# thanh-nt25/Whisper-context-biasing

Hardware: AMD Instinct MI355X
Metric: audio-seconds/sec (RTF) + biased-WER, whisper-small 30s clips, batch32 (higher is better)
Workload: dtype bf16

## Files before the change

### include/wcb.h

```cpp
#ifndef WCB_H_
#define WCB_H_
#include <stdint.h>

#ifdef __cplusplus
extern "C" {
#endif

typedef struct wcb_handle wcb_handle;
typedef struct wcb_bias wcb_bias;

enum wcb_status {
  WCB_OK = 0,
  WCB_ERR_ARG = -1,
  WCB_ERR_STATE = -2,
  WCB_ERR_HIP = -3,
  WCB_ERR_UNSUPPORTED = -4
};

enum wcb_dtype { WCB_BF16 = 0, WCB_F16 = 1, WCB_F32 = 2 };

typedef struct {
  int d_model, n_layers, n_heads, ffn, vocab, n_mel;
  int n_audio_ctx;
  int n_text_ctx;
// ... 47 lines not shown
int wcb_decode_info(wcb_handle* h, wcb_state* st, int32_t* max_new, int32_t* steps, int32_t* done);
int wcb_decode_result(wcb_handle* h, wcb_state* st, int32_t* out_ids, int out_ld, int32_t* out_steps, void* stream);
int wcb_decode_end(wcb_handle* h, wcb_state* st);

int wcb_synchronize(wcb_handle* h);

int wcb_forward(wcb_handle* h, const float* mel, int B, const int32_t* dec_ids, int T, float* logits,
                void* enc_out, void* stream);

int wcb_forward_enc(wcb_handle* h, const void* enc, int B, const int32_t* dec_ids, int T, float* logits, void* stream);

int wcb_forward_cached(wcb_handle* h, wcb_state* st, const int32_t* dec_ids, int T, float* logits, void* stream);

int wcb_bias_create(wcb_handle* h, const int32_t* tokens, const int32_t* offsets, int n_phrases,
                    const uint8_t* word_start, wcb_bias** out);
void wcb_bias_destroy(wcb_bias* b);
int wcb_bias_num_states(const wcb_bias* b);

int wcb_profile_enable(wcb_handle* h, int enable);
int wcb_profile_read(wcb_handle* h, int n, char (*names)[32], int64_t* launches, double* ms,
                     double* flops, double* bytes);

int wcb_profile_kernel(wcb_handle* h, int i, char* name, int cap, int64_t* grid);

int wcb_debug_copy(wcb_handle* h, const char* name, void* dst, int64_t bytes, int enc_layers);

int wcb_op_gemm(int dtype, const void* A, const void* W, int M, int N, int K, const float* bias, int act,
                const float* resid, void* out, int out_f32, void* stream);
int wcb_op_gemm_kernel(int dtype, const void* A, const void* W, int M, int N, int K, const float* bias, int act,
                       const float* resid, void* out, int out_f32, int kernel, void* stream);
int wcb_op_gemm_ln(int dtype, const float* X, const float* ln_w, const float* ln_b, const float* stats,
                   const void* W, int M, int N, int K, const float* bias, int act, void* out, int out_f32,
                   void* stream);
int wcb_op_layernorm(int dtype, const float* x, const float* w, const float* b, void* y, int M, int d,
                     void* stream);
int wcb_op_attention(int dtype, const void* q, const void* k, const void* v, void* o, int B, int H, int Sq,
                     int Sk, int flash, void* stream);
int wcb_op_attention_decode(int dtype, const void* q, const void* k, const void* v, void* o, int B, int H,
                            int Sk, int nsplit, int variant, void* stream);

int wcb_op_cross_attention_enc(int dtype, const void* q, const void* enc, const void* wkt, const void* wv,
                               const float* bv, void* o, int B, int H, int S, int nsplit, int variant, void* stream);

int wcb_op_weighted_ce(const float* logits, long ld, int B, int T, int V, const int32_t* labels,
                       const int32_t* spans, const int32_t* span_len, int N, int Lmax, float bias_weight,
                       float* per_token, float* loss, int32_t* count, void* stream);

int wcb_wer_counts(const char* const* refs, const char* const* hyps, int n, int64_t* errors, int64_t* ref_words,
                   int n_threads);
int wcb_bias_counts(const char* ref, const char* pred, const char* const* phrases, int n_phrases,
                    int64_t* distance, int64_t* tokens);

#ifdef __cplusplus
}
#endif
#endif
```

### whisper_context_biasing_amd/_lib.py

```python
from __future__ import annotations

import ctypes as C
import os
import subprocess

_HERE = os.path.dirname(os.path.abspath(__file__))
LIB_PATH = os.path.join(_HERE, "libwcb.so")
CSRC = os.path.join(_HERE, "csrc")

WCB_BF16, WCB_F16, WCB_F32 = 0, 1, 2
DTYPES = {"bf16": WCB_BF16, "f16": WCB_F16, "fp16": WCB_F16, "f32": WCB_F32, "fp32": WCB_F32}


class WcbModelDesc(C.Structure):
    _fields_ = [(n, C.c_int) for n in (
        "d_model", "n_layers", "n_heads", "ffn", "vocab", "n_mel", "n_audio_ctx", "n_text_ctx",
        "eos_token_id", "pad_token_id", "decoder_start_token_id", "dtype")]


class WcbGenCfg(C.Structure):
    _fields_ = [("max_new_tokens", C.c_int), ("min_new_tokens", C.c_int), ("num_beams", C.c_int),
                ("bias_boost", C.c_float), ("use_graph", C.c_int), ("async_out", C.c_int)]


# ... 15 lines not shown
    "wcb_generate": (C.c_int, [_P, _P, C.c_int, C.POINTER(WcbGenCfg), _P, _P, C.c_int, _P,
                               C.POINTER(C.c_int32), _P]),
    "wcb_synchronize": (C.c_int, [_P]),
    "wcb_decode_begin": (C.c_int, [_P, _P, C.c_int, C.c_int, _P, C.c_int, C.c_float, C.c_int, C.POINTER(_P), _P]),
    "wcb_decode_step": (C.c_int, [_P, _P, _P, _P, _P, _P]),
    "wcb_decode_end": (C.c_int, [_P, _P]),
    "wcb_decode_begin_beams": (C.c_int, [_P, _P, C.c_int, C.c_int, _P, C.c_int, C.c_int, C.c_float, C.c_int,
                                         C.POINTER(_P), _P]),
    "wcb_decode_parents": (C.c_int, [_P, _P, _P, _P]),
    "wcb_decode_info": (C.c_int, [_P, _P, C.POINTER(C.c_int32), C.POINTER(C.c_int32), C.POINTER(C.c_int32)]),
    "wcb_decode_result": (C.c_int, [_P, _P, _P, C.c_int, C.POINTER(C.c_int32), _P]),
    "wcb_forward": (C.c_int, [_P, _P, C.c_int, _P, C.c_int, _P, _P, _P]),
    "wcb_forward_enc": (C.c_int, [_P, _P, C.c_int, _P, C.c_int, _P, _P]),
    "wcb_forward_cached": (C.c_int, [_P, _P, _P, C.c_int, _P, _P]),
    "wcb_bias_create": (C.c_int, [_P, _P, _P, C.c_int, _P, C.POINTER(_P)]),
    "wcb_bias_destroy": (None, [_P]),
    "wcb_bias_num_states": (C.c_int, [_P]),
    "wcb_debug_copy": (C.c_int, [_P, C.c_char_p, _P, C.c_int64, C.c_int]),
    "wcb_profile_enable": (C.c_int, [_P, C.c_int]),
    "wcb_profile_read": (C.c_int, [_P, C.c_int, _P, _P, _P, _P, _P]),
    "wcb_profile_kernel": (C.c_int, [_P, C.c_int, C.c_char_p, C.c_int, C.POINTER(C.c_int64)]),
    "wcb_op_gemm": (C.c_int, [C.c_int, _P, _P, C.c_int, C.c_int, C.c_int, _P, C.c_int, _P, _P,
                              C.c_int, _P]),
    "wcb_op_gemm_kernel": (C.c_int, [C.c_int, _P, _P, C.c_int, C.c_int, C.c_int, _P, C.c_int, _P, _P,
                                     C.c_int, C.c_int, _P]),
    "wcb_op_gemm_ln": (C.c_int, [C.c_int, _P, _P, _P, _P, _P, C.c_int, C.c_int, C.c_int, _P, C.c_int, _P,
                                 C.c_int, _P]),
    "wcb_op_weighted_ce": (C.c_int, [_P, C.c_long, C.c_int, C.c_int, C.c_int, _P, _P, _P, C.c_int, C.c_int,
                                     C.c_float, _P, _P, _P, _P]),
    "wcb_wer_counts": (C.c_int, [C.POINTER(C.c_char_p), C.POINTER(C.c_char_p), C.c_int,
                                 C.POINTER(C.c_int64), C.POINTER(C.c_int64), C.c_int]),
    "wcb_bias_counts": (C.c_int, [C.c_char_p, C.c_char_p, C.POINTER(C.c_char_p), C.c_int,
                                  C.POINTER(C.c_int64), C.POINTER(C.c_int64)]),
    "wcb_op_layernorm": (C.c_int, [C.c_int, _P, _P, _P, _P, C.c_int, C.c_int, _P]),
    "wcb_op_attention_decode": (C.c_int, [C.c_int, _P, _P, _P, _P, C.c_int, C.c_int, C.c_int, C.c_int, C.c_int,
                                          _P]),
    "wcb_op_attention": (C.c_int, [C.c_int, _P, _P, _P, _P, C.c_int, C.c_int, C.c_int, C.c_int,
                                   C.c_int, _P]),
    "wcb_op_cross_attention_enc": (C.c_int, [C.c_int, _P, _P, _P, _P, _P, _P, C.c_int, C.c_int, C.c_int,
                                             C.c_int, C.c_int, _P]),
    "wcb_set_option": (C.c_int, [_P, C.c_char_p, C.c_int]),
}


class WcbError(RuntimeError):
    pass


class WcbArgError(WcbError, ValueError):
    """WCB_ERR_ARG: the reference raises ValueError for these (e.g. whisper_medical.py:87-90)."""


_lib = None


def build(force: bool = False, jobs: int = 8) -> str:
    if force or not os.path.exists(LIB_PATH):
        subprocess.run(["make", "-C", CSRC, f"-j{jobs}"], check=True)
    return LIB_PATH


def load() -> C.CDLL:
    global _lib
    if _lib is not None:
        return _lib
    if not os.path.exists(LIB_PATH):
# ... 19 lines not shown
```

### whisper_context_biasing_amd/csrc/gemm_impl.h

```cpp
#pragma once
#include <stdexcept>
#include <string>
#include "common.h"
#include "kernels.h"

#include <algorithm>
#include <cstdio>
#include <cstdlib>
#include <type_traits>

namespace wcb {

WCB_DEV void glds16(const void* gptr, void* lds_wave_base) {
  __builtin_amdgcn_global_load_lds(gptr, (__attribute__((address_space(3))) void*)lds_wave_base, 16, 0, 0);
}

WCB_DEV long a_row(const GemmArgs& g, int m) {
  return g.a_Mb ? (long)(m / g.a_Mb) * g.a_strideB + (long)(m % g.a_Mb) * g.lda : (long)m * g.lda;
}
WCB_DEV long c_row(const GemmArgs& g, int m) {
  return g.c_Mb ? (long)(m / g.c_Mb) * g.c_strideB + (long)(m % g.c_Mb) * g.ldc : (long)m * g.ldc;
}

enum : int { E_BIAS = 1, E_GELU = 2, E_RESID = 4, E_F32 = 8, E_ADDROW = 16, E_HEAD = 32, E_RUNTIME = 1 << 30 };
// ... 1960 lines not shown
#pragma unroll
    for (int e = 0; e < 8; ++e) {
      float v;
      if constexpr (__is_same(T, bf16_t)) v = bf16_to_f((bf16_t)a[ks][e]);
      else v = float(a[ks][e]);
      xv[ks][e] = v;
      s1 += v;
      s2 = fmaf(v, v, s2);
    }
  }
  s1 = xor16_add(s1); s2 = xor16_add(s2);
  s1 = xor32_add(s1); s2 = xor32_add(s2);
  if (lane < 16) rst[wave][lane] = float2{s1, s2};
  __syncthreads();
  s1 = 0.f; s2 = 0.f;
#pragma unroll
  for (int q = 0; q < NW; ++q) { const float2 t = rst[q][lane & 15]; s1 += t.x; s2 += t.y; }
  const float mean = s1 / K;
  const float rstd = rsqrtf(fmaxf(s2 / K - mean * mean, 0.f) + 1e-5f);
  if (r >= M) return;
#pragma unroll
  for (int ks = 0; ks < KPW; ++ks) {
    Frag o;
#pragma unroll
    for (int e = 0; e < 8; ++e) {
      const float gwe = e < 4 ? w[ks][0][e] : w[ks][1][e - 4], gbe = e < 4 ? b[ks][0][e] : b[ks][1][e - 4];
      const float v = (xv[ks][e] - mean) * rstd * gwe + gbe;
      o[e] = __builtin_bit_cast(typename std::remove_reference<decltype(o[0])>::type, DT<T>::fromf(v));
    }
    *reinterpret_cast<Frag*>(out + (long)r * K + kb + ks * 32) = o;
  }
}

template <typename T, int MF, int NW, int KPW, int AM>
static void launch_dec_k(const GemmArgs& g, hipStream_t s) {
  const int ntile = (g.N + 15) / 16, gy = (g.M + MF * 16 - 1) / (MF * 16);
  if (!g.sel_val && (AM == 3 || ntile * gy <= 1024)) {
    WCB_LAUNCH((gemm_dec_kernel<T, MF, NW, KPW, AM, false>), dim3(ntile, gy), dim3(NW * 64), 0, s, g);
  } else {
    const int gx = std::min(ntile, g.walkers > 0 ? g.walkers : kDecWalkers);
    int nw = 0, kpw = 0;
    if constexpr (sizeof(T) == 2 && AM != 3) {
      if (g.W_fm && lean_cfg(g.K, nw, kpw) && nw == NW && kpw == KPW) {
        if (AM == 2 && g.ln_scratch && g.sel_val && g.a_Mb == 0) {
          WCB_LAUNCH((ln_rows_kernel<T, NW, KPW>), dim3((g.M + 15) / 16), dim3(NW * 64), 0, s,
                     reinterpret_cast<const T*>(g.ln_a16), g.lda, g.ln_w, g.ln_b, reinterpret_cast<T*>(g.ln_scratch), g.M);
          GemmArgs h = g;
          h.A = g.ln_scratch; h.lda = g.K;
          h.ln_w = h.ln_b = nullptr; h.ln_a16 = nullptr; h.st_in = nullptr;
          WCB_LAUNCH((gemm_dec_kernel<T, MF, NW, KPW, 0, true, true>), dim3(gx, gy), dim3(NW * 64), 0, s, h);
          return;
        }
        WCB_LAUNCH((gemm_dec_kernel<T, MF, NW, KPW, AM, true, true>), dim3(gx, gy), dim3(NW * 64), 0, s, g);
        return;
      }
    }
    WCB_LAUNCH((gemm_dec_kernel<T, MF, NW, KPW, AM == 3 ? 0 : AM, true>), dim3(gx, gy), dim3(NW * 64), 0, s, g);
  }
}

template <typename T, int MF, int NW, int KPW>
static bool launch_dec_am(const GemmArgs& g, hipStream_t s) {
  constexpr int K = NW * KPW * 32;
  if (g.ln_w) {
    if constexpr (K <= 1280) {
      if (g.ln_a16) launch_dec_k<T, MF, NW, KPW, 2>(g, s);
      else launch_dec_k<T, MF, NW, KPW, 1>(g, s);
      return true;
    }
    return false;
  }
  if (g.a_grp_n) {
    if constexpr (K <= 1280) {
      launch_dec_k<T, MF, NW, KPW, 3>(g, s);
      return true;
    }
    return false;
  }
  launch_dec_k<T, MF, NW, KPW, 0>(g, s);
  return true;
}

template <typename T, int MF>
static bool launch_dec_mf(const GemmArgs& g, hipStream_t s) {
// ... 141 lines not shown
```

### whisper_context_biasing_amd/csrc/kernels.h

```cpp
#pragma once
#include <hip/hip_runtime.h>
#include <hip/hip_ext.h>
#include <stdint.h>

namespace wcb {

struct LaunchTimer {
  hipEvent_t start = nullptr, stop = nullptr;
  int n = 0;
  const void* fn = nullptr;
  long grid = 0;
};
inline thread_local LaunchTimer g_launch_timer;

#define WCB_LAUNCH(K, G, B, SH, S, ...)                                                              \
  do {                                                                                               \
    ::wcb::LaunchTimer& lt_ = ::wcb::g_launch_timer;                                                 \
    if (lt_.stop) {                                                                                  \
      if (!lt_.n) {                                                                                  \
        lt_.fn = reinterpret_cast<const void*>(K);                                                   \
        const dim3 g_ = dim3(G), b_ = dim3(B);                                                       \
        lt_.grid = (long)g_.x * g_.y * g_.z * b_.x * b_.y * b_.z;                                    \
      }                                                                                              \
      hipExtLaunchKernelGGL(K, G, B, SH, S, lt_.n ? nullptr : lt_.start, lt_.stop, 0, __VA_ARGS__);  \
// ... 22 lines not shown
  const int* pos = nullptr; int kv_T = 0;
  void* kv_out = nullptr; int n_split = 0;
  int kv_rps = 0;
  int tile = 0;
  const float* st_in = nullptr;
  float* st_out = nullptr;
  int st_nb = 0;
  float* sel_val = nullptr; int* sel_idx = nullptr;
  const uint32_t* sel_root_bits = nullptr; float sel_lam = 0.f;
  const int* sel_rowbase = nullptr;
  int sel_eos = -1; const int* sel_step = nullptr; int sel_min_new = 0;
  int a_grp_n = 0; long a_grp_off = 0;
  int skinny = 0;
  int ring_kt = 1;
  int wide = 0;
  int walkers = 0;
  void* out16 = nullptr;
  const void* ln_a16 = nullptr;
  const float* ln_u = nullptr;
  const float* ln_c = nullptr;
  const void* ln_wg = nullptr;
  const void* ln_wg_fm = nullptr;
  int lean_fold = 0;
  int lean_mf2 = 0;
  const void* xqk_wk = nullptr; void* xqk_out = nullptr; int xqk_nch = 0;
  const float* rst_in = nullptr; int rst_nb = 0;
  float* rst_out = nullptr;
  float clamp = 0.f;
  int lean = 0;
  const void* W_fm = nullptr;
  int c_fm = 0, a_fm = 0;
  void* out16_fm = nullptr;
  void* ln_scratch = nullptr;
  int raster = 0;
  int pp = 0;
  unsigned long long* kq_cnt = nullptr; int* kq_err = nullptr;
  const void* kq_w = nullptr; void* kq_out = nullptr; long kq_ld = 0;
  struct Stamp* lstamp = nullptr;
};

void gemm(DType t, const GemmArgs& g, hipStream_t s);
constexpr int kLnfMaxK = 1280;

void layernorm(DType t, const float* x, const float* w, const float* b, void* y, int M, int d,
               hipStream_t s);

void embed(DType t, const void* emb, const void* pos_emb, const int* ids, const int* pos, float* x,
           float* stats, int M, int d, hipStream_t s, void* x16 = nullptr, int V = 1 << 30, int rps = 1, int st_w = 16,
           void* x16fm = nullptr);
void prefill_ids(int* ids, const int* src, int R, int np, int ld, const int* pos, hipStream_t s);
void add_i32(int* p, int v, hipStream_t s);
constexpr int kDecWalkers = 512;
bool gemm_dec_supported(DType t, int K);
int lm_head_partials(DType t, int K, int vocab, int walkers = kDecWalkers);

constexpr int kStampSub = 64;
struct Stamp {
  unsigned long long* base = nullptr; const int* pos = nullptr; int stride = 0, idx = 0;
};

struct AttnArgs {
  const void* q = nullptr; long ldq = 0; long q_Sb = 0; int Sq = 1;
  const void* k = nullptr; const void* v = nullptr; long k_sb = 0, k_sh = 0, k_sk = 0;
  void* o = nullptr; long ldo = 0; long o_Sb = 0;
  int B = 0, H = 0;
  int nkeys = 0; const int* nkeys_dev = nullptr; int nkeys_add = 0;
// ... 140 lines not shown
```

### whisper_context_biasing_amd/csrc/runtime.cpp

```cpp
#include <hip/hip_runtime.h>

#include <algorithm>
#include <cxxabi.h>
#include <cmath>
#include <cstdio>
#include <cstring>
#include <map>
#include <thread>
#include <memory>
#include <stdexcept>
#include <string>
#include <vector>
#include <cstdlib>
#include <deque>
#include <atomic>

#include "../../include/wcb.h"
#include "kernels.h"

using namespace wcb;

namespace {

struct WcbError : std::runtime_error {
// ... 47 lines not shown
  float *lnx_w = nullptr, *lnx_b = nullptr;
  void* fc1_w = nullptr; float* fc1_b = nullptr;
  void* fc2_w = nullptr; float* fc2_b = nullptr;
  float *ln2_w = nullptr, *ln2_b = nullptr;
  void *qkv_wg = nullptr, *xq_wg = nullptr, *fc1_wg = nullptr;
  float *ln1_u = nullptr, *ln1_c = nullptr, *lnx_u = nullptr, *lnx_c = nullptr, *ln2_u = nullptr, *ln2_c = nullptr;
  void* xkt_w = nullptr; void* xv_w = nullptr; float* xv_b = nullptr;
  void *qkv_fm = nullptr, *o_fm = nullptr, *xq_fm = nullptr, *xkt_fm = nullptr, *xo_fm = nullptr, *fc1_fm = nullptr,
       *fc2_fm = nullptr;
  void* xv_fm = nullptr;
  void *qkv_wgfm = nullptr, *xq_wgfm = nullptr, *fc1_wgfm = nullptr;
};

struct ProfEntry {
  std::string name;
  int64_t launches = 0;
  double ms = 0, flops = 0, bytes = 0;
  const void* fn = nullptr;
  long grid = 0;
};

}

struct wcb_bias {
  int n_states = 1;
  int vocab = 0;
  uint64_t id = 0;
  wcb_handle* owner = nullptr;
  DevBuf root_bits, root_child, trans_off, trans_tok, trans_dst;
  DevBuf st_depth, st_keep;
};

static const char* const kLeanStampClass[] = {"dec_xattn", "dec_qkv", "dec_out", "dec_xq", "dec_xo", "dec_fc1", "dec_fc2",
                                              "dec_kq"};
static int lean_stamp_region(const char* cls) {
  for (int r = 1; r < 8; ++r)
    if (!strcmp(cls, kLeanStampClass[r])) return r;
  return 0;
}

struct DecCtx {
  static constexpr int kMaxSub = 8;
  hipStream_t hs = nullptr;
  hipStream_t sub[kMaxSub] = {};
  hipEvent_t ev_fork = nullptr, ev_join[kMaxSub] = {};
  int dec_B = 0, dec_T = 0;
  DevBuf kvself, dx, dx16, dx16fm, dh, dq, dqp, du, datt, dffn, dstats, drst, xpart, xml, xticket, logits, part_val, part_idx, ints,
      pids, outbuf, forced, beam;
  DevBuf kq_cnt;
  int nchunk = 64;
  hipGraphExec_t gexec = nullptr;
  hipGraphExec_t gexec_k = nullptr;
  int* done_h = nullptr;
  hipEvent_t ev_poll[2] = {};
  std::string gkey;
};

struct wcb_handle {
  wcb_model_desc d{};
  DType dt = kBF16;
  int device = 0;
  std::string err;
  hipStream_t he = nullptr;
  static constexpr int kMaxCtx = 4;
  int nctx = 2;
  hipEvent_t ev_xkv[kMaxCtx] = {}, ev_dec[kMaxCtx] = {};
  int gen_count = 0;
  hipEvent_t ev_in = nullptr, ev_out = nullptr;
  static constexpr int kMaxSub = DecCtx::kMaxSub;
  DecCtx dc[kMaxCtx];
  int n_sub = 1;
  int xsplit = 1;
  int xvariant = 0;
  int flash_split = 2;
  int beam_xattn = 0;
  int ln_fold = 1;
  int merge_v = 1;
  int xpart16 = 1;
  int xq_kq = 0;
  int ring_kt = 2;
  int beam_wide = 1;
  int beam_wfm = 0;
  int lean_fold = 1;
  int xqk = 1;
  int xqk_nch = 8;
  int merge_os = 1;
  int lm_walkers = 256;
  int mel_split = 0;
  int lean_mf2 = 0;
  int beam_chunks = 0;
  int beam_raster = 0;
  int lm_ln_split = 0;
  int enc_flash_qw = 4;
  int xmode = 1;
  int beam_xmode = 0;
  int group_rows = 512;
  int xenc_split = 6;
  int xenc_fm = 1;
  int xenc_variant = 1;
  int ln16 = 1;
  int vocab_pad = 0;
  int steps_per_graph = 8;
  int lean = 1;
  int lean_x = 1;
  struct wcb_state* step_state = nullptr;
  int enc_raster = 8;
  int enc_gemm = 4;
  bool dec_gemm = false;
  std::map<std::string, DevBuf> staged;
  std::vector<DevBuf> owned;
  bool ready = false;
  int dbg_enc_layers = -1;
  void *conv1_w = nullptr, *conv2_w = nullptr;
  float *conv1_b = nullptr, *conv2_b = nullptr, *enc_pos = nullptr;
  int k1pad = 0;
  std::vector<LayerW> enc, dec;
  float *enc_ln_w = nullptr, *enc_ln_b = nullptr, *dec_ln_w = nullptr, *dec_ln_b = nullptr;
  void* xkv_w = nullptr; float* xkv_b = nullptr;
  void *tok_emb = nullptr, *dec_pos = nullptr;
  void* tok_emb_fm = nullptr;
  DevBuf dft, dft3, mel_lo, mel_hi, mel_w, clip_max;
  int enc_B = 0;
  DevBuf xt, hbuf, x, h, qkv, att, ffn, encout;
  DevBuf xkv2[kMaxCtx];
  std::unique_ptr<wcb_bias> empty_bias;
  std::vector<wcb_bias*> biases;
  DevBuf dev_err;
  bool prof = false, prof_stamps = false;
  std::vector<ProfEntry> prof_e;
  std::deque<std::pair<int, std::pair<hipEvent_t, hipEvent_t>>> prof_pending;
  std::vector<hipEvent_t> ev_pool;
  DevBuf stamps, stamp_acc;
  static constexpr int kStampRegions = 8;
  unsigned long long* stamp_base(int buf, int region) {
    return stamps.as<unsigned long long>() + ((size_t)buf * kStampRegions + region) * stamp_slots() * 2 * kStampSub;
  }
  double xattn_bytes = 0, xattn_flops = 0;
  long stamp_slots() const { return (long)d.n_text_ctx * d.n_layers * kMaxSub; }

  int H() const { return d.n_heads; }
  int S() const { return d.n_audio_ctx; }

  void* upload(const void* src, size_t bytes) {
    owned.emplace_back();
    owned.back().ensure(bytes);
    HIPCHK(hipMemcpy(owned.back().p, src, bytes, hipMemcpyHostToDevice));
    return owned.back().p;
  }
  float* upload_f(const std::vector<float>& v) { return reinterpret_cast<float*>(upload(v.data(), v.size() * 4)); }
  void* own(size_t bytes) {
    owned.emplace_back();
    owned.back().ensure(bytes);
    return owned.back().p;
  }
  const float* W(const std::string& name, size_t expect) {
    auto it = staged.find(name);
    if (it == staged.end()) throw WcbError(WCB_ERR_STATE, "missing weight " + name);
    if (it->second.bytes != expect * 4)
      throw WcbError(WCB_ERR_ARG, "weight " + name + " has " + std::to_string(it->second.bytes / 4) +
                                      " elements, expected " + std::to_string(expect));
    return it->second.as<float>();
  }

  int prof_id(const char* name) {
    for (size_t i = 0; i < prof_e.size(); ++i)
      if (prof_e[i].name == name) return (int)i;
// ... 262 lines not shown
    REQUIRE(h && name, "bad argument");
    const std::string n = name;
    static const char* const kFreeWhileStepwise[] = {"decode_contexts", "enc_flash", "enc_gemm", "enc_raster",
                                                     "steps_per_graph", "kq_cnt_seed"};
    bool free_opt = false;
    for (const char* f : kFreeWhileStepwise) free_opt |= n == f;
    REQUIRE(free_opt || !h->step_state, "option " + n + ": a step-wise decode is active (wcb_decode_end first)");
    if (n == "xmode" || n == "beam_xmode") {
      REQUIRE(!h->ready, "option " + n + " selects the weight layouts: set it before wcb_finalize_weights");
      REQUIRE(value == 0 || value == 1, "option " + n + ": 0 or 1");
      if (n == "xmode") h->xmode = value && xenc_supported(h->dt, h->d.d_model);
      else h->beam_xmode = value && h->xmode;
      if (!h->xmode) h->beam_xmode = 0;
    } else if (n == "decode_contexts") {
      REQUIRE(value >= 1 && value <= wcb_handle::kMaxCtx, "option decode_contexts: 1..4");
      REQUIRE(!h->step_state || value < wcb_handle::kMaxCtx,
              "option decode_contexts: 4 while a step-wise decode is active (wcb_decode_end first)");
      h->nctx = value;
    } else if (n == "group_rows") {
      REQUIRE(value >= 16 && value <= 512, "option group_rows: 16..512");
      h->group_rows = value;
    } else if (n == "xenc_variant") {
      REQUIRE(value >= 0 && value <= 3, "option xenc_variant: 0..3");
      h->xenc_variant = value;
    } else if (n == "enc_flash") {
      REQUIRE(value == 2 || value == 4, "option enc_flash: 2 or 4");
      h->enc_flash_qw = value;
    } else if (n == "xenc_split") {
      REQUIRE(!h->ready, "option xenc_split: set before the weights are finalized");
      REQUIRE(value >= 1 && value <= kXencMaxSplit, "option xenc_split: 1..16");
      h->xenc_split = value;
    } else if (n == "lm_ln_split") {
      h->lm_ln_split = value != 0;
    } else if (n == "ring_kt") {
      REQUIRE(value == 1 || value == 2, "option ring_kt: 1 or 2");
      h->ring_kt = value;
    } else if (n == "kq_cnt_seed") {
      REQUIRE(value >= 0, "option kq_cnt_seed: >= 0");
      quiesce(h);
      for (DecCtx& D : h->dc) {
        if (!D.kq_cnt.p) continue;
        std::vector<unsigned long long> v(D.kq_cnt.bytes / 8, 4ull * (unsigned long long)value);
        HIPCHK(hipMemcpy(D.kq_cnt.p, v.data(), v.size() * 8, hipMemcpyHostToDevice));
      }
    } else if (n == "steps_per_graph") {
      REQUIRE(value >= 1 && value <= 64, "option steps_per_graph: 1..64");
      h->steps_per_graph = value;
    } else if (n == "xenc_fm") {
      h->xenc_fm = value != 0;
    } else if (n == "xq_kq") {
      h->xq_kq = value != 0;
    } else if (n == "enc_gemm") {
      REQUIRE(value == 0 || value == 1 || value == 4 || value == 5, "option enc_gemm: 0, 1, 4 or 5");
      h->enc_gemm = value;
    } else if (n == "enc_raster") {
      REQUIRE(value >= 0 && value <= 64, "option enc_raster: 0..64");
      h->enc_raster = value;
    } else if (n == "lean") {
      REQUIRE(!h->ready, "option lean selects weight layouts: set it before wcb_finalize_weights");
      h->lean = value != 0;
    } else if (n == "lean_x") {
      h->lean_x = value != 0;
    } else if (n == "xpart16") {
      h->xpart16 = value != 0;
    } else if (n == "merge_v") {
      h->merge_v = value != 0;
// ... 700 lines not shown
    xo.out16_fm = x16fm;
    proj("dec_xo", xo);
    const bool afm = fm_ok && w.fc1_fm && w.fc2_fm &&
                     (d == 512 || d == 768 || d == 1024 || d == 1280) &&
                     (h->d.ffn == 2048 || h->d.ffn == 3072 || h->d.ffn == 4096 || h->d.ffn == 5120);
    GemmArgs f1 = drow(x, d, w.fc1_w, M, h->d.ffn, d, dffn, h->d.ffn);
    f1.ln_w = w.ln2_w; f1.ln_b = w.ln2_b; f1.st_in = st; f1.st_nb = nbk; f1.ln_a16 = lna;
    f1.bias = w.fc1_b; f1.act = 1; f1.ln_u = w.ln2_u; f1.ln_c = w.ln2_c; f1.ln_wg = w.fc1_wg; f1.W_fm = w.fc1_fm; f1.ln_wg_fm = w.fc1_wgfm;
    f1.c_fm = afm;
    if (x16fm) { f1.ln_a16 = x16fm; f1.a_fm = 1; }
    proj("dec_fc1", f1);
    GemmArgs f2 = drow(dffn, h->d.ffn, w.fc2_w, M, d, h->d.ffn, x, d);
    f2.bias = w.fc2_b; f2.resid = x; f2.out_f32 = 1; f2.st_out = st_pub; f2.st_nb = nbk; f2.out16 = x16; f2.W_fm = w.fc2_fm;
    f2.a_fm = afm;
    f2.out16_fm = x16fm;
    proj("dec_fc2", f2);
  }
  if (c.lm_head) {
    GemmArgs lm = drow(x, d, h->tok_emb, M, h->d.vocab, d, c.logits_out + (size_t)b0 * c.logits_ld, c.logits_ld);
    if (rps > 1) { lm.ldc = h->d.vocab; lm.c_Mb = rps; lm.c_strideB = c.logits_ld; }
    const bool lm_tiled = tiled && rps == 1 && c.logits_ld >= h->vocab_pad;
    if (lm_tiled) lm.N = h->vocab_pad;
    lm.ln_w = h->dec_ln_w; lm.ln_b = h->dec_ln_b; lm.st_in = st; lm.st_nb = nbk; lm.ln_a16 = lna;
    if (h->lean) lm.W_fm = h->tok_emb_fm;
    if (h->lean && !tiled && rps == 1 && h->lm_ln_split) lm.ln_scratch = dh;
    lm.out_f32 = 1;
    if (c.select && !c.beam) {
      lm.walkers = h->lm_walkers;
      lm.sel_val = D.part_val.as<float>() + (size_t)b0 * D.nchunk;
      lm.sel_idx = D.part_idx.as<int>() + (size_t)b0 * D.nchunk;
      lm.sel_root_bits = c.bias->root_bits.as<uint32_t>(); lm.sel_lam = c.lam;
      lm.sel_rowbase = ints + I_NEXT + 3 * c.B + b0;
      lm.sel_eos = h->d.eos_token_id; lm.sel_step = ints + I_STEP; lm.sel_min_new = c.min_new;
    }
    if (lm_tiled) {
      proj("lm_head", lm);
    } else {
      dgemm(h, "lm_head", lm, st_);
    }
  }
}

void step_embed(wcb_handle* h, const StepCfg& c) {
  DecCtx& D = h->dc[c.buf];
  const int d = h->d.d_model, B = c.B;
  int* ints = D.ints.as<int>();
  const bool r32 = h->dec_gemm && lnf_possible(h);
  h->timed("dec_embed", 0, (double)B * d * (2.0 * esize(h->d.dtype) + 4), D.hs, [&] {
    embed(h->dt, h->tok_emb, h->dec_pos, ints + I_NEXT, ints + I_POS, D.dx.as<float>(),
          !h->dec_gemm ? D.dstats.as<float>() : r32 ? D.drst.as<float>() : nullptr, B, d, D.hs, D.dx16.p, h->d.vocab, 1,
          r32 ? 32 : 16, xfm_possible(h) ? D.dx16fm.p : nullptr);
  });
}

void decode_step(wcb_handle* h, const StepCfg& c) {
  DecCtx& D = h->dc[c.buf];
  const int d = h->d.d_model, B = c.B;
  int* ints = D.ints.as<int>();
  int* pos = ints + I_POS;
  int* next_ids = ints + I_NEXT;
  if (!c.embedded) step_embed(h, c);
  const int ngrp = (B + h->group_rows - 1) / h->group_rows;
  const int ns = std::max(ngrp, std::max(1, std::min(h->n_sub, B)));
  if (ns == 1 || !D.sub[0]) {
    for (int i = 0; i < ns; ++i) {
      const int b0 = (int)((long)B * i / ns), b1 = (int)((long)B * (i + 1) / ns);
// ... 870 lines not shown
    GemmArgs g = rowgemm(A, K, W, M, N, K, out, N);
    g.bias = bias; g.act = act; g.resid = resid; g.out_f32 = out_f32;
    g.raster = 8;
    if (kernel >= 6) {
      REQUIRE(M > 64 && dtype != WCB_F32, "decode-row tiles: 16-bit, M > 64");
      g.tile = 2; g.ring_kt = 2;
      if (kernel == 7) g.raster = 0;
      if (kernel <= 7 && wfm) g.W_fm = W;
      if (kernel > 7) {
        g.wide = kernel;
        if (wfm) g.W_fm = W;
        REQUIRE(!resid || resid == out, "wide tiles: the residual is updated in place (resid == out)");
      }
    } else {
      g.pp = kernel;
    }
    gemm(DType(dtype), g, (hipStream_t)stream);
    HIPCHK(hipGetLastError());
  });
}

int wcb_op_gemm(int dtype, const void* A, const void* W, int M, int N, int K, const float* bias, int act,
                const float* resid, void* out, int out_f32, void* stream) {
  return wcb_op_gemm_kernel(dtype, A, W, M, N, K, bias, act, resid, out, out_f32, 1, stream);
}

int wcb_op_gemm_ln(int dtype, const float* X, const float* ln_w, const float* ln_b, const float* stats,
                   const void* W, int M, int N, int K, const float* bias, int act, void* out, int out_f32, void* stream) {
  return guarded(nullptr, [&] {
    REQUIRE(X && ln_w && ln_b && stats && W && out && M > 0 && M <= 64 && N > 0 && K % 16 == 0, "bad argument");
    GemmArgs g = rowgemm(X, K, W, M, N, K, out, N);
    g.ln_w = ln_w; g.ln_b = ln_b; g.st_in = stats; g.st_nb = K / 16;
    g.bias = bias; g.act = act; g.out_f32 = out_f32;
    gemm(DType(dtype), g, (hipStream_t)stream);
    HIPCHK(hipGetLastError());
  });
}

int wcb_op_layernorm(int dtype, const float* x, const float* w, const float* b, void* y, int M, int d, void* stream) {
  return guarded(nullptr, [&] {
    REQUIRE(x && w && b && y && M > 0 && d > 0 && d % 64 == 0 && d <= 2048, "bad argument");
    layernorm(DType(dtype), x, w, b, y, M, d, (hipStream_t)stream);
    HIPCHK(hipGetLastError());
  });
}

int wcb_op_attention_decode(int dtype, const void* q, const void* k, const void* v, void* o, int B, int H, int Sk,
                            int nsplit, int variant, void* stream) {
  return guarded(nullptr, [&] {
    REQUIRE(q && k && v && o && B > 0 && H > 0 && Sk > 0 && Sk <= 2048 && nsplit >= 1 && nsplit <= 64, "bad argument");
    AttnArgs a;
    a.q = q; a.ldq = (long)H * 64; a.q_Sb = 1; a.Sq = 1;
    a.k = k; a.v = v; a.k_sb = (long)H * Sk * 64; a.k_sh = (long)Sk * 64; a.k_sk = 64;
    a.o = o; a.ldo = (long)H * 64; a.o_Sb = 1; a.B = B; a.H = H; a.nkeys = Sk;
    a.variant = variant;
    if (variant == 6 || variant == 7) a.kv_rows = Sk;
    int* nk_dev = nullptr;
    if (variant == 7) {
      HIPCHK(hipMallocAsync(reinterpret_cast<void**>(&nk_dev), 4, (hipStream_t)stream));
      const int nk1 = Sk - 1;
      write_i32(nk_dev, &nk1, 1, (hipStream_t)stream);
      a.nkeys_dev = nk_dev; a.nkeys_add = 1;
    }
    static DevBuf part, ticket;
    if (nsplit > 1) {
      a.nsplit = nsplit;
// ... 101 lines not shown
```

Measured before the change: 20400.

## Add streaming LM-head kernel with fused LayerNorm, bias boost and argmax select

Adds a dedicated lm_stream_kernel for the decoder LM head in greedy/select mode. It keeps the normalized activations in LDS, streams the vocab weight tiles with nontemporal loads through a multi-deep register ring, and fuses the bias boost, EOS masking and per-block argmax into the GEMM. The kernel is enabled by default through a new lm_stream option, and a standalone op entry point plus a profiling stamp region are added. The aim is to cut the memory-bound cost of reading the large vocab matrix each decode step. The cost is heavy register and LDS use, which may lower occupancy.

```diff
diff --git a/include/wcb.h b/include/wcb.h
--- a/include/wcb.h
+++ b/include/wcb.h
@@ -103,6 +103,10 @@
 int wcb_op_gemm_ln(int dtype, const float* X, const float* ln_w, const float* ln_b, const float* stats,
                    const void* W, int M, int N, int K, const float* bias, int act, void* out, int out_f32,
                    void* stream);
+int wcb_op_lm_head_select(int dtype, const void* A, const float* ln_w, const float* ln_b, void* ln_scratch,
+                          const void* W_fm, int M, int N, int K, const uint32_t* root_bits, const int32_t* rowbase,
+                          float lam, int eos, const int32_t* step, int min_new, int walkers, int kernel,
+                          float* part_val, int32_t* part_idx, float* logits, void* stream);
 int wcb_op_layernorm(int dtype, const float* x, const float* w, const float* b, void* y, int M, int d,
                      void* stream);
 int wcb_op_attention(int dtype, const void* q, const void* k, const void* v, void* o, int B, int H, int Sq,
diff --git a/whisper_context_biasing_amd/_lib.py b/whisper_context_biasing_amd/_lib.py
--- a/whisper_context_biasing_amd/_lib.py
+++ b/whisper_context_biasing_amd/_lib.py
@@ -71,6 +71,8 @@
                                  C.POINTER(C.c_int64), C.POINTER(C.c_int64), C.c_int]),
     "wcb_bias_counts": (C.c_int, [C.c_char_p, C.c_char_p, C.POINTER(C.c_char_p), C.c_int,
                                   C.POINTER(C.c_int64), C.POINTER(C.c_int64)]),
+    "wcb_op_lm_head_select": (C.c_int, [C.c_int, _P, _P, _P, _P, _P, C.c_int, C.c_int, C.c_int, _P, _P, C.c_float,
+                                        C.c_int, _P, C.c_int, C.c_int, C.c_int, _P, _P, _P, _P]),
     "wcb_op_layernorm": (C.c_int, [C.c_int, _P, _P, _P, _P, C.c_int, C.c_int, _P]),
     "wcb_op_attention_decode": (C.c_int, [C.c_int, _P, _P, _P, _P, C.c_int, C.c_int, C.c_int, C.c_int, C.c_int,
                                           _P]),
diff --git a/whisper_context_biasing_amd/csrc/gemm_impl.h b/whisper_context_biasing_amd/csrc/gemm_impl.h
--- a/whisper_context_biasing_amd/csrc/gemm_impl.h
+++ b/whisper_context_biasing_amd/csrc/gemm_impl.h
@@ -2016,6 +2016,264 @@
   }
 }
 
+template <typename T, int MF, int NW, int KPW, bool LN, int RD>
+__global__ __launch_bounds__(256) void lm_stream_kernel(GemmArgs g, Stamp lst) {
+  using Frag = typename DT<T>::frag;
+  const unsigned long long ts = lst.base ? stamp_now() : 0ull;
+  constexpr int WV = 4, NT = WV * 64, NKS = NW * KPW, K = NKS * 32, R = MF * 16;
+  extern __shared__ __attribute__((aligned(16))) char smem[];
+  Frag* afr = reinterpret_cast<Frag*>(smem);
+  float* lnp = reinterpret_cast<float*>(smem + MF * NKS * 1024);
+  float2* rst = reinterpret_cast<float2*>(smem + MF * NKS * 1024 + (LN ? 2 * K * 4 : 0));
+  float* selv = reinterpret_cast<float*>(rst + (LN ? NW * R : 0));
+  int* seli = reinterpret_cast<int*>(selv + WV * R);
+  const int tid = threadIdx.x, lane = tid & 63, wave = __builtin_amdgcn_readfirstlane(tid >> 6);
+  const int mb = blockIdx.y * R, gx = gridDim.x;
+  const int ntile = (g.N + 15) >> 4;
+  const bool mask_eos = *g.sel_step < g.sel_min_new;
+  const bool boost = g.sel_lam != 0.f;
+  const int t0 = blockIdx.x + wave * gx, tstep = WV * gx;
+  const int ntw = t0 < ntile ? (ntile - 1 - t0) / tstep + 1 : 0;
+  const T* Wf = reinterpret_cast<const T*>(g.W_fm) + lane * 8;
+  typedef const __attribute__((address_space(4))) uint32_t* CU32;
+  const CU32 rbp = (CU32)(unsigned long)(boost ? (const void*)g.sel_root_bits : g.W_fm);
+  auto load_tile = [&](Frag (&w)[NKS], int j) {
+    const bool own = j < ntw;
+    const T* p = own ? Wf + (long)(t0 + j * tstep) * (NKS * 512) : reinterpret_cast<const T*>(g.W_fm);
+#pragma unroll
+    for (int q = 0; q < NKS; ++q) w[q] = __builtin_nontemporal_load(reinterpret_cast<const Frag*>(p + q * 512));
+  };
+  constexpr int SPW = (NW + WV - 1) / WV;
+  constexpr int NQ = (NKS + WV - 1) / WV;
+  constexpr int LQ = LN ? (2 * K / 4 + NT - 1) / NT : 1;
+  Frag a[LN ? SPW : 1][MF][LN ? KPW : NQ];
+  f32x4 lq[LQ];
+  if constexpr (LN) {
+    const T* A0 = reinterpret_cast<const T*>(g.ln_a16);
+#pragma unroll
+    for (int sl = 0; sl < SPW; ++sl) {
+      const int v = wave + sl * WV;
+      if (v < NW) {
+        const int kb = v * (KPW * 32) + 8 * (lane >> 4);
+#pragma unroll
+        for (int i = 0; i < MF; ++i) {
+          const int m = min(mb + i * 16 + (lane & 15), g.M - 1);
+          const T* ap = A0 + (long)m * g.lda + kb;
+#pragma unroll
+          for (int ks = 0; ks < KPW; ++ks) a[sl][i][ks] = load_frag<T>(ap + ks * 32);
+        }
+      }
+    }
+#pragma unroll
+    for (int j = 0; j < LQ; ++j) {
+      const int c = (j * NT + tid) * 4;
+      lq[j] = c < 2 * K ? *reinterpret_cast<const f32x4*>((c < K ? g.ln_w : g.ln_b) + (c < K ? c : c - K))
+                        : f32x4{0.f, 0.f, 0.f, 0.f};
+    }
+  } else {
+    const T* A0 = reinterpret_cast<const T*>(g.A);
+#pragma unroll
+    for (int i = 0; i < MF; ++i) {
+      const int m = min(mb + i * 16 + (lane & 15), g.M - 1);
+      const T* ap = A0 + (long)m * g.lda + 8 * (lane >> 4);
+#pragma unroll
+      for (int n = 0; n < NQ; ++n) a[0][i][n] = load_frag<T>(ap + min(wave + n * WV, NKS - 1) * 32);
+    }
+  }
+  int rbase[MF][4];
+#pragma unroll
+  for (int i = 0; i < MF; ++i)
+#pragma unroll
+    for (int e = 0; e < 4; ++e) {
+      const int row = mb + i * 16 + (lane >> 4) * 4 + e;
+      rbase[i][e] = (boost && row < g.M) ? g.sel_rowbase[row] : 0;
+    }
+  __builtin_amdgcn_sched_barrier(0);
+  Frag w[RD][NKS];
+#pragma unroll
+  for (int d = 0; d < RD; ++d) load_tile(w[d], d);
+  __builtin_amdgcn_sched_barrier(0);
+  if constexpr (LN) {
+#pragma unroll
+    for (int j = 0; j < LQ; ++j) {
+      const int c = (j * NT + tid) * 4;
+      if (c < 2 * K) *reinterpret_cast<f32x4*>(lnp + c) = lq[j];
+    }
+    auto xv = [&](int sl, int i, int ks, int e) -> float {
+      if constexpr (__is_same(T, bf16_t)) return bf16_to_f((bf16_t)a[sl][i][ks][e]);
+      else return float(a[sl][i][ks][e]);
+    };
+#pragma unroll
+    for (int sl = 0; sl < SPW; ++sl) {
+      const int v = wave + sl * WV;
+      if (v < NW) {
+#pragma unroll
+        for (int i = 0; i < MF; ++i) {
+          float s1 = 0.f, s2 = 0.f;
+#pragma unroll
+          for (int ks = 0; ks < KPW; ++ks) {
+#pragma unroll
+            for (int e = 0; e < 8; ++e) {
+              const float x = xv(sl, i, ks, e);
+              s1 += x;
+              s2 = fmaf(x, x, s2);
+            }
+          }
+          s1 = xor16_add(s1); s2 = xor16_add(s2);
+          s1 = xor32_add(s1); s2 = xor32_add(s2);
+          if (lane < 16) rst[v * R + i * 16 + lane] = float2{s1, s2};
+        }
+      }
+    }
+    __syncthreads();
+#pragma unroll
+    for (int i = 0; i < MF; ++i) {
+      float s1 = 0.f, s2 = 0.f;
+#pragma unroll
+      for (int q = 0; q < NW; ++q) { const float2 t = rst[q * R + i * 16 + (lane & 15)]; s1 += t.x; s2 += t.y; }
+      const float mean = s1 / K;
+      const float rstd = rsqrtf(fmaxf(s2 / K - mean * mean, 0.f) + 1e-5f);
+#pragma unroll
+      for (int sl = 0; sl < SPW; ++sl) {
+        const int v = wave + sl * WV;
+        if (v < NW) {
+          const int kb = v * (KPW * 32) + 8 * (lane >> 4);
+#pragma unroll
+          for (int ks = 0; ks < KPW; ++ks) {
+            const f32x4 w0 = *reinterpret_cast<const f32x4*>(lnp + kb + ks * 32);
+            const f32x4 w1 = *reinterpret_cast<const f32x4*>(lnp + kb + ks * 32 + 4);
+            const f32x4 b0 = *reinterpret_cast<const f32x4*>(lnp + K + kb + ks * 32);
+            const f32x4 b1 = *reinterpret_cast<const f32x4*>(lnp + K + kb + ks * 32 + 4);
+            Frag o;
+#pragma unroll
+            for (int e = 0; e < 8; ++e) {
+              const float gw = e < 4 ? w0[e] : w1[e - 4], gb = e < 4 ? b0[e] : b1[e - 4];
+              const float x = (xv(sl, i, ks, e) - mean) * rstd * gw + gb;
+              o[e] = __builtin_bit_cast(typename std::remove_reference<decltype(o[0])>::type, DT<T>::fromf(x));
+            }
+            afr[(i * NKS + v * KPW + ks) * 64 + lane] = o;
+          }
+        }
+      }
+    }
+  } else {
+#pragma unroll
+    for (int i = 0; i < MF; ++i)
+#pragma unroll
+      for (int n = 0; n < NQ; ++n)
+        if (wave + n * WV < NKS) afr[(i * NKS + wave + n * WV) * 64 + lane] = a[0][i][n];
+  }
+  __syncthreads();
+
+  float best[MF][4];
+  int bi[MF][4];
+#pragma unroll
+  for (int i = 0; i < MF; ++i)
+#pragma unroll
+    for (int e = 0; e < 4; ++e) { best[i][e] = -INFINITY; bi[i][e] = 0x7fffffff; }
+  const Frag* al = afr + lane;
+  float* lg = reinterpret_cast<float*>(g.out);
+  for (int j0 = 0; j0 < ntw; j0 += RD) {
+#pragma unroll
+    for (int d = 0; d < RD; ++d) {
+      const int j = j0 + d;
+      if (j >= ntw) goto walked;
+      const int ct = t0 + j * tstep;
+      const uint32_t rbw = rbp[boost ? ct >> 1 : 0];
+      f32x4 acc[MF][NW];
+#pragma unroll
+      for (int v = 0; v < NW; ++v)
+#pragma unroll
+        for (int i = 0; i < MF; ++i) acc[i][v] = f32x4{0.f, 0.f, 0.f, 0.f};
+      constexpr int PF = NKS < 4 ? NKS : 4;
+      Frag ab[PF + 1][MF];
+      auto read_a = [&](int s) {
+        const int q = (s % NW) * KPW + s / NW;
+#pragma unroll
+        for (int i = 0; i < MF; ++i) ab[s % (PF + 1)][i] = al[(i * NKS + q) * 64];
+      };
+#pragma unroll
+      for (int s = 0; s < PF; ++s) read_a(s);
+#pragma unroll
+      for (int s = 0; s < NKS; ++s) {
+        if (s + PF < NKS) read_a(s + PF);
+        const int v = s % NW, q = v * KPW + s / NW;
+#pragma unroll
+        for (int i = 0; i < MF; ++i) acc[i][v] = mma16(ab[s % (PF + 1)][i], w[d][q], acc[i][v]);
+        __builtin_amdgcn_sched_barrier(0);
+      }
+      load_tile(w[d], j + RD);
+      __builtin_amdgcn_sched_barrier(0);
+      const int nn = ct * 16 + (lane & 15);
+      const int bit = (int)((rbw >> (nn & 31)) & 1u);
+#pragma unroll
+      for (int i = 0; i < MF; ++i)
+#pragma unroll
+        for (int e = 0; e < 4; ++e) {
+          float x = 0.f;
+#pragma unroll
+          for (int v = 0; v < NW; ++v) x += acc[i][v][e];
+          if (lg) {
+            const int row = mb + i * 16 + (lane >> 4) * 4 + e;
+            if (row < g.M && nn < g.N) lg[(long)row * g.ldc + nn] = x;
+          }
+          if (boost) x = bias_bonus(x, g.sel_lam, rbase[i][e] + bit);
+          if (mask_eos && nn == g.sel_eos) x = -INFINITY;
+          if (nn < g.N && x > best[i][e]) { best[i][e] = x; bi[i][e] = nn; }
+        }
+    }
+  }
+walked:
+#pragma unroll
+  for (int i = 0; i < MF; ++i)
+#pragma unroll
+    for (int e = 0; e < 4; ++e) {
+      float x = best[i][e];
+      int xi = bi[i][e];
+#pragma unroll
+      for (int o = 1; o < 16; o <<= 1) {
+        const float ov = __shfl_xor(x, o, 64);
+        const int oi = __shfl_xor(xi, o, 64);
+        if (ov > x || (ov == x && oi < xi)) { x = ov; xi = oi; }
+      }
+      if ((lane & 15) == 0) {
+        selv[wave * R + i * 16 + (lane >> 4) * 4 + e] = x;
+        seli[wave * R + i * 16 + (lane >> 4) * 4 + e] = xi;
+      }
+    }
+  __syncthreads();
+  if (tid < R && mb + tid < g.M) {
+    float x = selv[tid];
+    int xi = seli[tid];
+#pragma unroll
+    for (int q = 1; q < WV; ++q) {
+      const float ov = selv[q * R + tid];
+      const int oi = seli[q * R + tid];
+      if (ov > x || (ov == x && oi < xi)) { x = ov; xi = oi; }
+    }
+    g.sel_val[(long)(mb + tid) * gx + blockIdx.x] = x;
+    g.sel_idx[(long)(mb + tid) * gx + blockIdx.x] = xi;
+  }
+  if (lst.base && tid == 0) stamp_commit(lst, ts);
+}
+
+template <typename T, int MF, int NW, int KPW, bool LN>
+static void launch_lm_stream(const GemmArgs& g, int gx, int gy, hipStream_t s) {
+  constexpr int NKS = NW * KPW, K = NKS * 32, R = MF * 16;
+  constexpr int RD = 3 * NKS <= 63 ? 3 : 2;
+  constexpr int lds = MF * NKS * 1024 + (LN ? 2 * K * 4 + NW * R * 8 : 0) + 4 * R * 8;
+  static_assert(lds <= 160 * 1024, "LDS budget");
+  static bool attr_set = false;
+  if (!attr_set) {
+    (void)hipFuncSetAttribute((const void*)lm_stream_kernel<T, MF, NW, KPW, LN, RD>,
+                              hipFuncAttributeMaxDynamicSharedMemorySize, lds);
+    attr_set = true;
+  }
+  Stamp lst;
+  if (g.lstamp) lst = *g.lstamp;
+  WCB_LAUNCH((lm_stream_kernel<T, MF, NW, KPW, LN, RD>), dim3(gx, gy), dim3(256), lds, s, g, lst);
+}
+
 template <typename T, int MF, int NW, int KPW, int AM>
 static void launch_dec_k(const GemmArgs& g, hipStream_t s) {
   const int ntile = (g.N + 15) / 16, gy = (g.M + MF * 16 - 1) / (MF * 16);
@@ -2026,14 +2284,30 @@
     int nw = 0, kpw = 0;
     if constexpr (sizeof(T) == 2 && AM != 3) {
       if (g.W_fm && lean_cfg(g.K, nw, kpw) && nw == NW && kpw == KPW) {
+        constexpr int K = NW * KPW * 32;
+        constexpr bool kStream = (AM == 0 || AM == 2) && (K == 64 || K == 512 || K == 768 || K == 1024 || K == 1280);
+        const bool stream = kStream && g.lm_stream && g.sel_val && (!g.out || g.out_f32) && g.a_Mb == 0 && g.c_Mb == 0 &&
+                            !g.bias && !g.resid && !g.act && !g.mode && !g.st_out && !g.out16;
         if (AM == 2 && g.ln_scratch && g.sel_val && g.a_Mb == 0) {
           WCB_LAUNCH((ln_rows_kernel<T, NW, KPW>), dim3((g.M + 15) / 16), dim3(NW * 64), 0, s,
                      reinterpret_cast<const T*>(g.ln_a16), g.lda, g.ln_w, g.ln_b, reinterpret_cast<T*>(g.ln_scratch), g.M);
           GemmArgs h = g;
           h.A = g.ln_scratch; h.lda = g.K;
           h.ln_w = h.ln_b = nullptr; h.ln_a16 = nullptr; h.st_in = nullptr;
+          if constexpr (kStream) {
+            if (stream) {
+              launch_lm_stream<T, MF, NW, KPW, false>(h, gx, gy, s);
+              return;
+            }
+          }
           WCB_LAUNCH((gemm_dec_kernel<T, MF, NW, KPW, 0, true, true>), dim3(gx, gy), dim3(NW * 64), 0, s, h);
           return;
+        }
+        if constexpr (kStream) {
+          if (stream) {
+            launch_lm_stream<T, MF, NW, KPW, AM == 2>(g, gx, gy, s);
+            return;
+          }
         }
         WCB_LAUNCH((gemm_dec_kernel<T, MF, NW, KPW, AM, true, true>), dim3(gx, gy), dim3(NW * 64), 0, s, g);
         return;
diff --git a/whisper_context_biasing_amd/csrc/kernels.h b/whisper_context_biasing_amd/csrc/kernels.h
--- a/whisper_context_biasing_amd/csrc/kernels.h
+++ b/whisper_context_biasing_amd/csrc/kernels.h
@@ -78,6 +78,7 @@
   int c_fm = 0, a_fm = 0;
   void* out16_fm = nullptr;
   void* ln_scratch = nullptr;
+  int lm_stream = 0;
   int raster = 0;
   int pp = 0;
   unsigned long long* kq_cnt = nullptr; int* kq_err = nullptr;
diff --git a/whisper_context_biasing_amd/csrc/runtime.cpp b/whisper_context_biasing_amd/csrc/runtime.cpp
--- a/whisper_context_biasing_amd/csrc/runtime.cpp
+++ b/whisper_context_biasing_amd/csrc/runtime.cpp
@@ -103,7 +103,8 @@
 };
 
 static const char* const kLeanStampClass[] = {"dec_xattn", "dec_qkv", "dec_out", "dec_xq", "dec_xo", "dec_fc1", "dec_fc2",
-                                              "dec_kq"};
+                                              "dec_kq", "lm_head"};
+constexpr int kLmStampRegion = 8;
 static int lean_stamp_region(const char* cls) {
   for (int r = 1; r < 8; ++r)
     if (!strcmp(cls, kLeanStampClass[r])) return r;
@@ -162,6 +163,7 @@
   int beam_chunks = 0;
   int beam_raster = 0;
   int lm_ln_split = 0;
+  int lm_stream = 1;
   int enc_flash_qw = 4;
   int xmode = 1;
   int beam_xmode = 0;
@@ -202,7 +204,7 @@
   std::deque<std::pair<int, std::pair<hipEvent_t, hipEvent_t>>> prof_pending;
   std::vector<hipEvent_t> ev_pool;
   DevBuf stamps, stamp_acc;
-  static constexpr int kStampRegions = 8;
+  static constexpr int kStampRegions = 9;
   unsigned long long* stamp_base(int buf, int region) {
     return stamps.as<unsigned long long>() + ((size_t)buf * kStampRegions + region) * stamp_slots() * 2 * kStampSub;
   }
@@ -531,6 +533,8 @@
       h->xenc_split = value;
     } else if (n == "lm_ln_split") {
       h->lm_ln_split = value != 0;
+    } else if (n == "lm_stream") {
+      h->lm_stream = value != 0;
     } else if (n == "ring_kt") {
       REQUIRE(value == 1 || value == 2, "option ring_kt: 1 or 2");
       h->ring_kt = value;
@@ -1297,6 +1301,14 @@
       lm.sel_root_bits = c.bias->root_bits.as<uint32_t>(); lm.sel_lam = c.lam;
       lm.sel_rowbase = ints + I_NEXT + 3 * c.B + b0;
       lm.sel_eos = h->d.eos_token_id; lm.sel_step = ints + I_STEP; lm.sel_min_new = c.min_new;
+      if (h->lm_stream && h->lean && h->dec_gemm && h->dt != kF32 && !tiled && rps == 1 && lm.W_fm && lm.ln_a16) {
+        lm.lm_stream = 1;
+        if (h->prof_stamps) {
+          lst.base = h->stamp_base(c.buf, kLmStampRegion);
+          lst.pos = pos; lst.stride = L * wcb_handle::kMaxSub; lst.idx = chain;
+          lm.lstamp = &lst;
+        }
+      }
     }
     if (lm_tiled) {
       proj("lm_head", lm);
@@ -2233,6 +2245,32 @@
     GemmArgs g = rowgemm(X, K, W, M, N, K, out, N);
     g.ln_w = ln_w; g.ln_b = ln_b; g.st_in = stats; g.st_nb = K / 16;
     g.bias = bias; g.act = act; g.out_f32 = out_f32;
+    gemm(DType(dtype), g, (hipStream_t)stream);
+    HIPCHK(hipGetLastError());
+  });
+}
+
+int wcb_op_lm_head_select(int dtype, const void* A, const float* ln_w, const float* ln_b, void* ln_scratch,
+                          const void* W_fm, int M, int N, int K, const uint32_t* root_bits, const int32_t* rowbase,
+                          float lam, int eos, const int32_t* step, int min_new, int walkers, int kernel,
+                          float* part_val, int32_t* part_idx, float* logits, void* stream) {
+  return guarded(nullptr, [&] {
+    int nw = 0, kpw = 0;
+    REQUIRE(A && W_fm && step && part_val && part_idx && M > 0 && M <= 64 && N > 0, "bad argument");
+    REQUIRE(dtype == WCB_BF16 || dtype == WCB_F16, "16-bit dtypes only");
+    REQUIRE(lean_cfg(K, nw, kpw) && gemm_dec_supported(DType(dtype), K), "K: 64, 512, 768, 1024 or 1280");
+    REQUIRE(!ln_w == !ln_b && (!ln_scratch || ln_w), "LayerNorm: gamma and beta together; the scratch only with them");
+    REQUIRE(lam == 0.f || (root_bits && rowbase), "the boost needs root bits and row bases");
+    REQUIRE(walkers == 128 || walkers == 192 || walkers == 256 || walkers == 384 || walkers == 512 || walkers == 1024,
+            "walkers: 128, 192, 256, 384, 512 or 1024");
+    REQUIRE(kernel == 0 || kernel == 1, "kernel: 0 (gemm_dec_kernel's walker) or 1 (lm_stream_kernel)");
+    GemmArgs g = rowgemm(A, K, W_fm, M, N, K, logits, N);
+    g.W_fm = W_fm; g.out_f32 = 1;
+    if (ln_w) { g.ln_w = ln_w; g.ln_b = ln_b; g.ln_a16 = A; g.ln_scratch = ln_scratch; }
+    g.walkers = walkers; g.lm_stream = kernel;
+    g.sel_val = part_val; g.sel_idx = part_idx;
+    g.sel_root_bits = root_bits; g.sel_rowbase = rowbase; g.sel_lam = lam;
+    g.sel_eos = eos; g.sel_step = step; g.sel_min_new = min_new;
     gemm(DType(dtype), g, (hipStream_t)stream);
     HIPCHK(hipGetLastError());
   });
```

Result: no change. 20230 (-0.8%).
